# mnhrk15/integrated_path_planning

Hardware: AMD Instinct MI355X
Metric: candidate trajectories/sec (higher is better)
Workload: dtype f64; 1 GPU; config4: 256 ego instances/GPU x 2240-candidate lattice (5 s, dt 0.1 s), 20-sample x 30-pedestrian x 51-step fp32 prediction distribution (layout [S][P][T][2]), eps=0; 8 distinct batches rotated (501 MB of obstacle tensors per GPU); instances_per_gpu=256, instances_total=256, rotation_batches=8, plan_calls_in_flight=4

## Files before the change

### integrated_path_planning_amd/csrc/fot_kernels.hip

```cpp
#include <hip/hip_runtime.h>

#include <cstdlib>
#include <cstring>

#include "fot_math.hpp"
#include "fot_kernels.h"

namespace fot {


template <int CTRL, int ROW_MASK>
__device__ __forceinline__ float dpp_f32(float v)
{
    return __int_as_float(__builtin_amdgcn_update_dpp(__float_as_int(v), __float_as_int(v), CTRL, ROW_MASK, 0xf, false));
}

#define FOT_WAVE_REDUCE_F32(NAME, OP)                                                        \
    __device__ __forceinline__ float NAME(float v)                                           \
    {                                                                                        \
        v = OP(v, dpp_f32<0xB1, 0xf>(v));                           \
        v = OP(v, dpp_f32<0x4E, 0xf>(v));                           \
        v = OP(v, dpp_f32<0x141, 0xf>(v));                              \
        v = OP(v, dpp_f32<0x140, 0xf>(v));                                   \
        v = OP(v, dpp_f32<0x142, 0xa>(v));                     \
        v = OP(v, dpp_f32<0x143, 0xc>(v));                     \
        return __int_as_float(__builtin_amdgcn_readlane(__float_as_int(v), 63));             \
    }
FOT_WAVE_REDUCE_F32(wave_min_f32, fminf)
FOT_WAVE_REDUCE_F32(wave_max_f32, fmaxf)


__device__ __forceinline__ ScanBest wave_argmin(ScanBest b)
{
#pragma unroll
    for (int off = 32; off >= 1; off >>= 1) {
        ScanBest o;
        o.dist = __shfl_xor(b.dist, off, WAVE);
        o.idx = __shfl_xor(b.idx, off, WAVE);
        scan_merge(b, o);
    }
    return b;
}

template <typename T>
__device__ __forceinline__ T load_const(const T *table, int i)
{
    static_assert(sizeof(T) % sizeof(uint64_t) == 0, "copied in 8-byte words");
#if defined(__HIP_DEVICE_COMPILE__)
    typedef const __attribute__((address_space(4))) uint64_t const_u64;
    const_u64 *src = (const_u64 *)(table + i);
    T v;
#pragma unroll
    for (int k = 0; k < (int)(sizeof(T) / sizeof(uint64_t)); ++k) ((uint64_t *)&v)[k] = src[k];
    return v;
#else
    return table[i];
#endif
}

extern __shared__ double s_spl[];
constexpr int SPLINE_LDS_KNOTS = 512;

__device__ __forceinline__ void stage_spline_copy(const SplineView &g, double *s_spl)
{
    const double *src[9] = { g.s, g.ax, g.bx, g.cx, g.dx, g.ay, g.by, g.cy, g.dy };
    for (int i = threadIdx.x; i < 9 * g.n; i += blockDim.x) {
        const int a = i / g.n, j = i - a * g.n;
        s_spl[i] = src[a][j];
    }
}

__device__ __forceinline__ SplineView staged_spline_view(const SplineView &g, double *s_spl)
{
    SplineView l = g;
    l.s = s_spl; l.ax = s_spl + g.n; l.bx = s_spl + 2 * g.n; l.cx = s_spl + 3 * g.n; l.dx = s_spl + 4 * g.n;
    l.ay = s_spl + 5 * g.n; l.by = s_spl + 6 * g.n; l.cy = s_spl + 7 * g.n; l.dy = s_spl + 8 * g.n;
    return l;
}

__device__ __forceinline__ SplineView stage_spline(const SplineView &g, int lds_knots, double *s_spl = fot::s_spl)
{
    if (g.n > lds_knots) return g;
    stage_spline_copy(g, s_spl);
    __syncthreads();
    return staged_spline_view(g, s_spl);
}

__device__ __forceinline__ void refine_apply(int outcome, double s_end, double &s, double &ds)
{
    if (outcome == 0) s = fmax(0.0, s - ds);
    else if (outcome == 1) s = fmin(s_end, s + ds);
    else ds *= 0.5;
}

__device__ __forceinline__ double refine_nearest_wave(const SplineView &sp, double x, double y, double best_s, int lane)
{
    const double s_end = sp.s[sp.n - 1];
    int depth = 0, o1 = 0, o2 = 0, pos = lane;
    if (lane >= 12) { const int i = lane - 12; depth = 2; o1 = i / 9; o2 = (i / 3) % 3; pos = i % 3; }
    else if (lane >= 3) { const int i = lane - 3; depth = 1; o1 = i / 3; pos = i % 3; }
    if (lane >= 39) { depth = 0; pos = 1; }
    double ds = 0.2;
    for (int it = 0; it < 20; it += 3) {
        double ms = best_s, mds = ds;
        if (depth >= 1) refine_apply(o1, s_end, ms, mds);
        if (depth >= 2) refine_apply(o2, s_end, ms, mds);
        const double probe = pos == 0 ? fmax(0.0, ms - mds) : (pos == 1 ? ms : fmin(s_end, ms + mds));
        double px, py;
        spline_xy(sp, probe, px, py);
        const double dist = hypot_cr(x - px, y - py);
        const int rounds = 20 - it < 3 ? 20 - it : 3;
        int base = 0, r1 = 0;
// ... 1051 lines not shown
    if ((int)blockIdx.x < a.n_inst) {
        select_instance_wave((int)blockIdx.x, (int)threadIdx.x);
        record_written((int)blockIdx.x, (int)threadIdx.x);
    }
}

#define FOT_EVAL_LEAN false
#define FOT_EVAL_KERNEL(name) name
#include "fot_eval_kernels.inc"
#undef FOT_EVAL_LEAN
#undef FOT_EVAL_KERNEL
#define FOT_EVAL_LEAN true
#define FOT_EVAL_KERNEL(name) name##_lean
#include "fot_eval_kernels.inc"
#undef FOT_EVAL_LEAN
#undef FOT_EVAL_KERNEL


#ifndef FOT_CULL_KG
#define FOT_CULL_KG 4
#endif
constexpr int CULL_KG = FOT_CULL_KG;
constexpr int CULL_LIST = 256;
constexpr int CULL_PBOX = 96;
constexpr uint32_t CULL_IDX_MASK = 0xFFFFFu;
constexpr int CULL_VER = 256;
constexpr int CULL_BAD = 32;
constexpr uint32_t CULL_DEAD = 0xFFFFFFFFu;

template <typename T, int KG>
__device__ __forceinline__ void
cull_group(const DevParams *__restrict__ Pp, const InstDesc *__restrict__ desc, const InstState *__restrict__ state,
           const SplineView &sp, double *dyn_lds, const T *__restrict__ static_xy, const T *__restrict__ dyn_xy,
           int32_t *__restrict__ ent_cnt, f2 *__restrict__ ent32, d2 *__restrict__ ent64, uint8_t *__restrict__ ent_sid,
           TileStep *__restrict__ wave_rng, const int32_t *__restrict__ tile_cand0, const int32_t *__restrict__ tile_n,
           const int32_t *__restrict__ tile_span, const uint8_t *__restrict__ nan_flag, int ablate, int inst, int k0)
{
    __shared__ int s_cnt[KG][CULL_BINS + 1];
    __shared__ int s_start[KG][CULL_BINS + 1];
    __shared__ int s_nin[KG];
    __shared__ uint32_t s_list[KG][CULL_LIST];
    __shared__ uint32_t s_ver[CULL_VER];
    __shared__ uint32_t s_bad[CULL_BAD];
    __shared__ int s_nver, s_nbad;
    __shared__ Box32 s_box[KG];
    __shared__ BinMap s_bm[KG];
    __shared__ float s_margin[KG];
    __shared__ Box32 s_pbox[KG][CULL_PBOX];
    __shared__ LonQuartic s_linfo[CULL_PBOX];
    __shared__ uint8_t s_lext[CULL_PBOX];
    const DevParams &P = *Pp;
    const int n_ext_cap = P.n_ti + P.n_brake;
    double *s_ext = dyn_lds;
    double *s_latq = s_ext + KG * n_ext_cap * 2;
    const InstDesc &D = desc[inst];
    const InstState &S = state[inst];
    if (D.ent_cap == 0) return;
    const int tid = threadIdx.x, lane = tid & (WAVE - 1);
    const int wv = __builtin_amdgcn_readfirstlane(tid / WAVE);
    const int nk = P.n_total - k0 < KG ? P.n_total - k0 : KG;
    const int n_grid_lon = P.n_ti * D.n_tv;
    const int n_prof = S.c2f_ok ? n_grid_lon + S.n_brake : 0;
    const double sq_dyn = D.dyn_mode == FOT_DYN_SINGLE ? P.sq_r_dyn : P.sq_r;
    const double sq_max = sq_dyn > P.sq_r ? sq_dyn : P.sq_r;
    const FilterConst fc = filter_const(sq_max, sq_dyn < P.sq_r ? sq_dyn : P.sq_r);
    const float slack = box_footprint_slack(P);
    const int n_ext = P.n_ti + (S.c2f_ok ? S.n_brake : 0);
    for (int w = tid; w < n_prof && w < CULL_PBOX; w += KG * WAVE) {
        s_linfo[w] = lon_quartic(profile_info(P, D, S.frenet0, w, false));
        s_lext[w] = (uint8_t)extent_index(P, D, w);
    }
    if (S.c2f_ok && tid < n_ext) {
        const bool brake = tid >= P.n_ti;
        lateral_extent_coeffs(P, S.frenet0, brake, brake ? P.brake[tid - P.n_ti] : P.ti[tid], s_latq + tid * 9);
    }
    __syncthreads();
    if (ablate & 16) return;

    struct Raw { T x, y; };
    const bool dyn_on = D.dyn_mode != FOT_DYN_NONE;
    const int n_dyn = dyn_on ? D.S * D.P : 0;
    const int total = D.n_static + n_dyn;
    const bool tmajor = D.dyn_tmajor != 0;

    const int kl = tmajor ? wv : (lane & (KG - 1));
    const int i_first = tmajor ? lane : wv * (WAVE / KG) + lane / KG;
    constexpr int STRIDE = WAVE;
    const int row_l = k0 + kl < D.T - 1 ? k0 + kl : D.T - 1;
    auto fetch = [&](int i, Raw &o) {
        const int ic = i < total ? i : total - 1;
        const int j = ic - D.n_static;
        const T *ps = static_xy + 2 * ((int64_t)D.static_off + ic);
        const T *pd = dyn_xy + 2 * (D.dyn_off + (tmajor ? (int64_t)row_l * n_dyn + j : (int64_t)j * D.T + row_l));
        const Raw *src = (const Raw *)(ic < D.n_static ? ps : pd);
        o = *src;
    };
    if (!(ablate & 8)) {
        for (int i = tid; i < nk * n_ext; i += KG * WAVE) {
            const int ks = i / n_ext, e = i - ks * n_ext;
            const bool brake = e >= P.n_ti;
            const int n_eval = brake ? P.brake[e - P.n_ti].n_t : P.ti[e].n_t;
            double *ext = s_ext + (ks * n_ext_cap + e) * 2;
            lateral_extent_q(s_latq + e * 9, brake, k0 + ks, n_eval, P.dt, ext[0], ext[1]);
        }
        __syncthreads();
        const int n_tab = n_prof < CULL_PBOX ? n_prof : CULL_PBOX;
        for (int i = tid; i < nk * n_tab; i += KG * WAVE) {
            const int ks = i / n_tab, w = i - ks * n_tab;
            const double *ext = s_ext + (ks * n_ext_cap + s_lext[w]) * 2;
            s_pbox[ks][w] = profile_box_from(s_linfo[w], D, sp, k0 + ks, P.dt, ext[0], ext[1]);
        }
        __syncthreads();
    }
    {
        Box32 bw = box_empty();
        if (wv < nk && !(ablate & 8)) {
            for (int w = lane; w < n_prof; w += WAVE) {
                if (w < CULL_PBOX) {
                    box_merge(bw, s_pbox[wv][w]);
                } else {
                    const double *ext = s_ext + (wv * n_ext_cap + extent_index(P, D, w)) * 2;
                    box_merge(bw, profile_box_at(P, D, S.frenet0, sp, w, k0 + wv, ext[0], ext[1]));
                }
            }
        }
        bw.x0 = wave_min_f32(bw.x0); bw.y0 = wave_min_f32(bw.y0);
        bw.x1 = wave_max_f32(bw.x1); bw.y1 = wave_max_f32(bw.y1);
        const float mw = cull_margin(sq_max, bw) + slack;
        if (lane == 0) { s_box[wv] = bw; s_margin[wv] = mw; s_bm[wv] = bin_map(bw, mw); s_nin[wv] = 0; }
        if (lane <= CULL_BINS) s_cnt[wv][lane] = 0;
        if (tid == 0) { s_nver = 0; s_nbad = 0; }
    }
    __syncthreads();

    const bool lazy = dyn_on && !tmajor && !(ablate & 128);
    const Raw *tracks = (const Raw *)(dyn_xy + 2 * D.dyn_off);
    auto track_has_nan = [&](int j) {
        bool bad = false;
        for (int t = 0; t < D.T; ++t) { const Raw p = tracks[(int64_t)j * D.T + t]; bad |= (p.x != p.x) | (p.y != p.y); }
        return bad;
    };
    auto track_bad = [&](int i) {
        if (i < D.n_static) return false;
        return lazy ? track_has_nan(i - D.n_static) : nan_flag[D.nan_off + (i - D.n_static)] != 0;
    };

    {
        const Box32 bl = s_box[kl];
        const float ml = s_margin[kl];
        const BinMap bml = s_bm[kl];
        const bool live_l = kl < nk && bl.x0 <= bl.x1 && !(ablate & 4);
        auto classify = [&](int i, const Raw &o) {
            const float fx = (float)((double)o.x - D.ego.x), fy = (float)((double)o.y - D.ego.y);
            const bool in = i < total && live_l && cull_inside(bl, ml, fx, fy);
            if (lazy) {
                const uint64_t m = __ballot(in && i >= D.n_static);
                if ((lane & (KG - 1)) == 0 && ((m >> lane) & ((1ull << KG) - 1ull)) != 0ull) {
                    const int v = atomicAdd(&s_nver, 1);
                    if (v < CULL_VER) s_ver[v] = (uint32_t)i;
                }
                if (in) {
                    const int j = atomicAdd(&s_nin[kl], 1);
                    if (j < CULL_LIST) s_list[kl][j] = (uint32_t)i | ((uint32_t)bin_of(bml, fx, fy) << 20);
                }
                return;
            }
            if (in) {
                if (i >= D.n_static && nan_flag[D.nan_off + (i - D.n_static)]) return;
                const int bin = bin_of(bml, fx, fy);
                atomicAdd(&s_cnt[kl][bin], 1);
                const int j = atomicAdd(&s_nin[kl], 1);
                if (j < CULL_LIST) s_list[kl][j] = (uint32_t)i | ((uint32_t)bin << 20);
            }
        };
#ifndef FOT_CULL_UNROLL
#define FOT_CULL_UNROLL 4
#endif
        constexpr int UNROLL = FOT_CULL_UNROLL;
        if (ablate & 64) {
        } else if (D.n_static == 0) {
            const char *p0 = (const char *)(dyn_xy + 2 * (D.dyn_off + (tmajor ? (int64_t)row_l * n_dyn + i_first
                                                                              : (int64_t)i_first * D.T + row_l)));
            const int64_t step = (int64_t)(tmajor ? STRIDE : STRIDE * D.T) * (int64_t)(2 * sizeof(T));
            const char *p = p0;
            for (int ib = i_first; ib < total; ib += UNROLL * STRIDE) {
                Raw o[UNROLL];
#pragma unroll
                for (int u = 0; u < UNROLL; ++u) {
                    o[u] = *(const Raw *)(ib + u * STRIDE < total ? p : p0);
                    p += step;
                }
#pragma unroll
                for (int u = 0; u < UNROLL; ++u) classify(ib + u * STRIDE, o[u]);
            }
        } else {
            for (int ib = i_first; ib < total; ib += UNROLL * STRIDE) {
                Raw o[UNROLL];
#pragma unroll
                for (int u = 0; u < UNROLL; ++u) fetch(ib + u * STRIDE, o[u]);
#pragma unroll
                for (int u = 0; u < UNROLL; ++u) classify(ib + u * STRIDE, o[u]);
            }
        }
    }
    __syncthreads();
    if (lazy) {
#ifndef FOT_CULL_VU
#define FOT_CULL_VU 4
#endif
        constexpr int VU = FOT_CULL_VU;
        const int n_ver = s_nver < CULL_VER ? s_nver : CULL_VER;
        for (int v0 = wv; v0 < n_ver; v0 += VU * KG) {
            Raw p[VU];
#pragma unroll
            for (int u = 0; u < VU; ++u) {
                const int v = v0 + u * KG < n_ver ? v0 + u * KG : v0;
                p[u] = tracks[(int64_t)((int)s_ver[v] - D.n_static) * D.T + (lane < D.T ? lane : D.T - 1)];
            }
#pragma unroll
            for (int u = 0; u < VU; ++u) {
                const int v = v0 + u * KG;
                if (v >= n_ver) break;
                bool bad = (p[u].x != p[u].x) | (p[u].y != p[u].y);
                for (int t = WAVE + lane; t < D.T; t += WAVE) {
                    const Raw q = tracks[(int64_t)((int)s_ver[v] - D.n_static) * D.T + t];
                    bad |= (q.x != q.x) | (q.y != q.y);
                }
                if (__ballot(bad) != 0ull && lane == 0) {
                    const int nb = atomicAdd(&s_nbad, 1);
                    if (nb < CULL_BAD) s_bad[nb] = s_ver[v];
                }
            }
        }
        __syncthreads();
    }
    if (wv >= nk) return;
    const int kk = wv, k = k0 + wv;
    const bool listed = !lazy || (s_nin[kk] <= CULL_LIST && s_nver <= CULL_VER && s_nbad <= CULL_BAD);
    const Box32 bk = s_box[kk];
    const BinMap bmk = s_bm[kk];
    const float mk = s_margin[kk];
    const bool live_k = bk.x0 <= bk.x1;
    const int row = k < D.T - 1 ? k : D.T - 1;
    auto point = [&](int i, d2 &o, int &sid) {
        sid = SID_STATIC;
        if (i < D.n_static) {
            const int64_t in = D.static_off + i;
            o.x = (double)static_xy[2 * in]; o.y = (double)static_xy[2 * in + 1];
        } else {
            const int j = i - D.n_static;
            const int64_t in = D.dyn_off + (tmajor ? (int64_t)row * n_dyn + j : (int64_t)j * D.T + row);
            o.x = (double)dyn_xy[2 * in]; o.y = (double)dyn_xy[2 * in + 1];
            sid = j / D.P;
        }
    };
    if (lazy) {
        if (listed) {
            const int n_bad = s_nbad;
            for (int j = lane; j < s_nin[kk]; j += WAVE) {
                const uint32_t e = s_list[kk][j];
                bool bad = false;
                for (int b = 0; b < n_bad; ++b) bad |= s_bad[b] == (e & CULL_IDX_MASK);
                if (bad) s_list[kk][j] = CULL_DEAD;
                else atomicAdd(&s_cnt[kk][e >> 20], 1);
            }
        } else {
            for (int i0 = 0; i0 < total; i0 += WAVE) {
                const int i = i0 + lane;
                if (i >= total) continue;
                d2 o; int sid;
                point(i, o, sid);
                const float fx = (float)(o.x - D.ego.x), fy = (float)(o.y - D.ego.y);
                if (live_k && cull_inside(bk, mk, fx, fy) && !track_bad(i)) atomicAdd(&s_cnt[kk][bin_of(bmk, fx, fy)], 1);
            }
        }
        __builtin_amdgcn_fence(__ATOMIC_SEQ_CST, "wavefront");
        __builtin_amdgcn_wave_barrier();
    }
    {
        const int c = lane < CULL_BINS ? s_cnt[kk][lane] : 0;
        int incl = c;
#pragma unroll
        for (int off = 1; off < WAVE; off <<= 1) {
            const int t = __shfl_up(incl, off, WAVE);
            if (lane >= off) incl += t;
        }
        if (lane <= CULL_BINS) { s_start[kk][lane] = incl - c; s_cnt[kk][lane] = incl - c; }
    }
    __builtin_amdgcn_fence(__ATOMIC_SEQ_CST, "wavefront");
    __builtin_amdgcn_wave_barrier();
    const int64_t base = D.ent_off + (int64_t)k * D.ent_cap;
    TileStep *rng = wave_rng + (int64_t)D.tile0 * P.n_total + k;
    const int count = s_start[kk][CULL_BINS];
    if (lazy ? listed : count <= CULL_LIST) {
        for (int j = lane; j < ((ablate & 2) ? 0 : (lazy ? s_nin[kk] : count)); j += WAVE) {
            const uint32_t e = s_list[kk][j];
            if (e == CULL_DEAD) continue;
            const int i = (int)(e & CULL_IDX_MASK), bin = (int)(e >> 20);
            d2 o; int sid;
            point(i, o, sid);
            const int pos = atomicAdd(&s_cnt[kk][bin], 1);
            ent32_store(ent32, base + pos, (float)(o.x - D.ego.x), (float)(o.y - D.ego.y));
            ent64[base + pos] = o;
            ent_sid[base + pos] = (uint8_t)sid;
        }
    } else {
        for (int i0 = 0; i0 < total; i0 += WAVE) {
            const int i = i0 + lane;
            if (i >= total) continue;
            d2 o; int sid;
            point(i, o, sid);
            const float fx = (float)(o.x - D.ego.x), fy = (float)(o.y - D.ego.y);
            if (live_k && cull_inside(bk, mk, fx, fy) && !track_bad(i)) {
                const int bin = bin_of(bmk, fx, fy);
                const int pos = atomicAdd(&s_cnt[kk][bin], 1);
                ent32_store(ent32, base + pos, fx, fy);
                ent64[base + pos] = o;
                ent_sid[base + pos] = (uint8_t)sid;
            }
        }
    }
    const int padded = (count + 2 * ENT_CHUNK - 1) & ~(2 * ENT_CHUNK - 1);
    if (lane < padded - count) {
        d2 o; o.x = INFINITY; o.y = INFINITY;
        ent32_store(ent32, base + count + lane, FAR32, FAR32);
        ent64[base + count + lane] = o;
        ent_sid[base + count + lane] = SID_STATIC;
    }
    if (lane == 0) ent_cnt[(int64_t)inst * P.n_total + k] = padded;
    for (int w = lane; w < D.n_tiles; w += WAVE) {
        TileStep r = { 0u, 0.0f, 0.0f, 0u };
        const int idx0 = tile_cand0[D.shape_off + w];
        if (live_k && idx0 < S.n_cand && tile_n[D.shape_off + w] > 0 && !(ablate & 1)) {
            const uint32_t sp01 = (uint32_t)tile_span[D.shape_off + w];
            const int s0 = (int)(sp01 >> 16), s1 = (int)(sp01 & 0xffffu) < n_prof - 1 ? (int)(sp01 & 0xffffu) : n_prof - 1;
            Box32 wb = box_empty();
            for (int sl = s0; sl <= s1; ++sl) {
                if (sl < CULL_PBOX) { box_merge(wb, s_pbox[kk][sl]); continue; }
                const double *ext = s_ext + (kk * n_ext_cap + extent_index(P, D, sl)) * 2;
                box_merge(wb, profile_box_at(P, D, S.frenet0, sp, sl, k, ext[0], ext[1]));
            }
            const float wm = cull_margin(sq_max, wb) + slack;
            r.rng = strip_range(bmk, wb, wm, [&](int bb) { return s_start[kk][bb]; });
            box_thresholds(fc, wb, wm, r.thr, r.thr_sure);
        }
        rng[(int64_t)w * P.n_total] = r;
    }
}

template <typename T>
__global__ void __launch_bounds__(CULL_KG * WAVE)
k_cull(const DevParams *__restrict__ Pp, const InstDesc *__restrict__ desc, const InstState *__restrict__ state,
       int n_inst, SplineView sp_hbm, const SplineView *__restrict__ sp_table, int mixed, int lds_knots,
       const T *__restrict__ static_xy, const T *__restrict__ dyn_xy,
       int32_t *__restrict__ ent_cnt, f2 *__restrict__ ent32, d2 *__restrict__ ent64, uint8_t *__restrict__ ent_sid,
       TileStep *__restrict__ wave_rng, const int32_t *__restrict__ tile_cand0, const int32_t *__restrict__ tile_n,
       const int32_t *__restrict__ tile_span, const uint8_t *__restrict__ nan_flag,
       int ablate)
{
    if (ablate & 32) return;
    const int groups = (Pp->n_total + CULL_KG - 1) / CULL_KG;
    const int xcd = blockIdx.x & 7, seq = blockIdx.x >> 3;
    const int inst = xcd + 8 * (seq / groups), k0 = (seq % groups) * CULL_KG;
    if (inst >= n_inst) return;
    if (mixed) { Pp += desc[inst].scen; sp_hbm = load_const(sp_table, desc[inst].scen); }
    const SplineView sp = stage_spline(sp_hbm, lds_knots);
    cull_group<T, CULL_KG>(Pp, desc, state, sp, s_spl + 9 * lds_knots, static_xy, dyn_xy, ent_cnt, ent32, ent64, ent_sid,
                           wave_rng, tile_cand0, tile_n, tile_span, nan_flag, ablate, inst, k0);
}
// ... 309 lines not shown
```

### integrated_path_planning_amd/csrc/fot_math.hpp

```cpp
#pragma once

#include <math.h>
#include "fot_types.h"

namespace fot {


FOT_HD double fast_rcp(double a)
{
#if defined(__HIP_DEVICE_COMPILE__)
    double x = __builtin_amdgcn_rcp(a);
    x = fma(x, fma(-a, x, 1.0), x);
#ifdef FOT_NEWTON2
    x = fma(x, fma(-a, x, 1.0), x);
#endif
    return x;
#else
    return 1.0 / a;
#endif
}

FOT_HD double fast_rsqrt(double a)
{
#if defined(__HIP_DEVICE_COMPILE__)
// ... 879 lines not shown
    d1 = d0;
    if (!brake) {
        lat_coeffs(fr, (double)(P.n_di - 1 - P.n_side) * P.d_road_w, ti, q);
        lat_sample(q, k, n_eval, P.dt, d1, u0, u1, u2);
    }
}

FOT_HD void lateral_extent_q(const double *q9, bool brake, int k, int n_eval, double dt, double &d0, double &d1)
{
    double u0, u1, u2;
    lat_sample(q9, k, n_eval, dt, d0, u0, u1, u2);
    d1 = d0;
    if (!brake) {
        const double q_hi[6] = { q9[0], q9[1], q9[2], q9[6], q9[7], q9[8] };
        lat_sample(q_hi, k, n_eval, dt, d1, u0, u1, u2);
    }
}

FOT_HD void lateral_extent_coeffs(const DevParams &P, const double *fr, bool brake, const TimeInfo &ti, double *q9)
{
    double q_hi[6];
    lat_coeffs(fr, brake ? fr[3] : -(double)P.n_side * P.d_road_w, ti, q9);
    lat_coeffs(fr, brake ? fr[3] : (double)(P.n_di - 1 - P.n_side) * P.d_road_w, ti, q_hi);
    q9[6] = q_hi[3]; q9[7] = q_hi[4]; q9[8] = q_hi[5];
}

FOT_HD Box32 segment_box(double rx, double ry, double cos_r, double sin_r, double d0, double d1, double ox, double oy)
{
    Box32 b = box_empty();
    const double x0 = rx - sin_r * d0, y0 = ry + cos_r * d0, x1 = rx - sin_r * d1, y1 = ry + cos_r * d1;
    if (x0 == x0 && y0 == y0) box_add(b, (float)(x0 - ox), (float)(y0 - oy));
    if (x1 == x1 && y1 == y1) box_add(b, (float)(x1 - ox), (float)(y1 - oy));
    return b;
}

FOT_HD Box32 profile_box(const DevParams &P, const double *fr, bool brake, const TimeInfo &ti, const LonSample &ls,
                         int k, int n_eval, double ox, double oy)
{
    double d0, d1;
    lateral_extent(P, fr, brake, ti, k, n_eval, d0, d1);
    return segment_box(ls.rx, ls.ry, ls.cos_r, ls.sin_r, d0, d1, ox, oy);
}

FOT_HD Box32 profile_box_at(const DevParams &P, const InstDesc &D, const double *fr, const SplineView &sp, int slot,
                            int k, double d0, double d1)
{
    const LonInfo L = profile_info(P, D, fr, slot, false);
    if (k >= L.n_t) return box_empty();
    double s_, u0, u1, u2;
    lon_sample(L, k, P.dt, s_, u0, u1, u2);
    SplinePt p;
    spline_point(sp, s_, p);
    const double inv = fast_rsqrt(p.dx * p.dx + p.dy * p.dy);
    return segment_box(p.x, p.y, p.dx * inv, p.dy * inv, d0, d1, D.ego.x, D.ego.y);
}

struct LonQuartic {
    double a0, a1, a2, a3, a4;
    int32_t n_t, n_eval;
};

FOT_HD LonQuartic lon_quartic(const LonInfo &L)
{
    LonQuartic q;
    q.a0 = L.a0; q.a1 = L.a1; q.a2 = L.a2; q.a3 = L.a3; q.a4 = L.a4; q.n_t = L.n_t; q.n_eval = L.n_eval;
    return q;
}

FOT_HD Box32 profile_box_from(const LonQuartic &Q, const InstDesc &D, const SplineView &sp, int k, double dt, double d0,
                              double d1)
{
    if (k >= Q.n_t) return box_empty();
    LonInfo L;
    L.a0 = Q.a0; L.a1 = Q.a1; L.a2 = Q.a2; L.a3 = Q.a3; L.a4 = Q.a4; L.n_t = Q.n_t; L.n_eval = Q.n_eval;
    L.Js = 0.0; L.sd_last = 0.0; L.T = 0.0;
    double s_, u0, u1, u2;
    lon_sample(L, k, dt, s_, u0, u1, u2);
    SplinePt p;
    spline_point(sp, s_, p);
    const double inv = fast_rsqrt(p.dx * p.dx + p.dy * p.dy);
    return segment_box(p.x, p.y, p.dx * inv, p.dy * inv, d0, d1, D.ego.x, D.ego.y);
}

FOT_HD int extent_index(const DevParams &P, const InstDesc &D, int slot)
{
    const int n_grid_lon = P.n_ti * D.n_tv;
    return slot < n_grid_lon ? slot / D.n_tv : P.n_ti + (slot - n_grid_lon);
}

FOT_HD float box_footprint_slack(const DevParams &P)
{
    float m = 0.0f;
    if (P.has_footprint)
        for (int c = 0; c < P.n_circ; ++c) m = fmaxf(m, (float)fabs(P.circ_off[c]) * 1.000001f);
    return m;
}

constexpr int CULL_BINS = 32;
constexpr int ENT_CHUNK_ = 8;

struct BinMap {
    int axis;
    float lo, inv_w;
};

FOT_HD BinMap bin_map(const Box32 &b, float margin)
{
    BinMap m;
    m.axis = (b.y1 - b.y0) > (b.x1 - b.x0) ? 1 : 0;
    const float lo = (m.axis ? b.y0 : b.x0) - margin, hi = (m.axis ? b.y1 : b.x1) + margin;
    m.lo = lo;
    m.inv_w = (float)CULL_BINS / fmaxf(hi - lo, 1e-6f);
    return m;
}

FOT_HD int bin_of_value(const BinMap &m, float v)
{
    const float t = (v - m.lo) * m.inv_w;
    return t >= (float)(CULL_BINS - 1) ? CULL_BINS - 1 : (t > 0.0f ? (int)t : 0);
}

FOT_HD int bin_of(const BinMap &m, float x, float y) { return bin_of_value(m, m.axis ? y : x); }

template <class StartFn>
FOT_HD uint32_t strip_range(const BinMap &m, const Box32 &wb, float margin, const StartFn &bin_start)
{
    if (!(wb.x0 <= wb.x1)) return 0u;
    const float lo = (m.axis ? wb.y0 : wb.x0) - margin, hi = (m.axis ? wb.y1 : wb.x1) + margin;
    const int b_lo = bin_of_value(m, lo), b_hi = bin_of_value(m, hi);
    const int e_lo = bin_start(b_lo), e_hi = bin_start(b_hi + 1);
    if (e_hi <= e_lo) return 0u;
    const int c_lo = e_lo / ENT_CHUNK_, c_hi = (e_hi + ENT_CHUNK_ - 1) / ENT_CHUNK_;
    return ((uint32_t)c_lo << 16) | (uint32_t)c_hi;
}

FOT_HD void wave_profile_span(const DevParams &P, const InstDesc &D, int n_tv_grid_lon, int idx0, int idx1,
                              int &first, int &last)
{
    const int per_prof = P.n_di;
    first = idx0 < D.n_grid ? idx0 / per_prof : n_tv_grid_lon + (idx0 - D.n_grid);
    last = idx1 < D.n_grid ? idx1 / per_prof : n_tv_grid_lon + (idx1 - D.n_grid);
}

constexpr int ENT_CHUNK = 8;
static_assert(ENT_CHUNK == 8, "strip_range assumes 8-entry chunks");
constexpr int SID_STATIC = 255;
struct alignas(64) f2x8 { float x[ENT_CHUNK]; float y[ENT_CHUNK]; };

FOT_HD void ent32_store(f2 *e32, int64_t pos, float x, float y)
{
    f2x8 *c = (f2x8 *)e32 + (pos >> 3);
    c->x[pos & 7] = x;
    c->y[pos & 7] = y;
}

FOT_HD float min_sqdist32_8(const f2x8 &c, float fx, float fy)
{
    float t[ENT_CHUNK];
    for (int j = 0; j < ENT_CHUNK; ++j) {
        const float dx = fx - c.x[j], dy = fy - c.y[j];
        t[j] = fmaf(dy, dy, dx * dx);
    }
    float m = fminf(fminf(t[0], t[1]), t[2]);
    m = fminf(fminf(m, t[3]), t[4]);
    m = fminf(fminf(m, t[5]), t[6]);
    return fminf(m, t[7]);
}

struct FilterConst { float sq, r, sq_lo; };

FOT_HD FilterConst filter_const(double sq, double sq_min)
// ... 472 lines not shown
```

### integrated_path_planning_amd/csrc/fot_setup.hpp

```cpp
#pragma once

#include <algorithm>
#include <cmath>
#include <cstring>
#include <string>
#include <cstdlib>
#include <vector>

#include "fot_types.h"
#include "fot_math.hpp"

namespace fot {


inline bool time_info(double T, double dt, TimeInfo &ti)
{
    ti.T = T;
    ti.n_t = (int)std::nearbyint(T / dt) + 1;
    if (ti.n_t < 1 || ti.n_t > FOT_MAX_NT) return false;
    const double T2 = T * T, T3 = T2 * T, T4 = T2 * T2, T5 = T4 * T;
    {
        const double a = 3.0 * T2, b = 4.0 * T3, c = 6.0 * T, d = 12.0 * T2;
        const double det = a * d - b * c;
        ti.qa[0] = d / det; ti.qa[1] = -b / det; ti.qa[2] = -c / det; ti.qa[3] = a / det;
// ... 331 lines not shown
    L.n_inst = b.n_inst;
    L.desc.resize(b.n_inst);
    L.grouped = sc[0].shapes->grouped;
    for (int s = 0; s < n_scen; ++s)
        if (sc[s].shapes->row_budget > L.row_budget) L.row_budget = sc[s].shapes->row_budget;
    std::vector<uint8_t> used((size_t)n_scen, 0);
    for (int i = 0; i < b.n_inst; ++i) {
        InstDesc &D = L.desc[i];
        D = InstDesc();
        D.ego = b.ego[i];
        const int si = scen ? scen[i] : 0;
        if (si < 0 || si >= n_scen) { err = "unknown scenario id"; return FOT_ERR_INVALID; }
        const fot_params &hp = *sc[si].hp;
        const DevParams &P = *sc[si].P;
        const TileShapes &shapes = *sc[si].shapes;
        D.scen = si;
        used[(size_t)si] = 1;
        if (D.ego.has_prev_s < 0 || D.ego.has_prev_s > FOT_EGO_IS_FRENET) { err = "has_prev_s must be 0 .. 3"; return FOT_ERR_INVALID; }
        if (i == 0 && D.ego.has_prev_s == FOT_PREV_S_CHAINED) { err = "the first instance cannot be chained"; return FOT_ERR_INVALID; }
        if (i > 0 && D.ego.has_prev_s == FOT_PREV_S_CHAINED && si != L.desc[i - 1].scen) {
            err = "a chained instance must be on its predecessor's scenario (a chain is one planner)"; return FOT_ERR_INVALID;
        }
        const double target = b.target_speed[i];
        D.target_speed = target;
        D.max_stop = b.max_stop_distance ? b.max_stop_distance[i] : NAN;
        D.lim_speed = hp.max_speed; D.lim_accel = hp.max_accel; D.lim_curv = hp.max_curvature; D.lim_lat = hp.max_lat_accel;
        if (b.overrides) {
            const fot_overrides &o = b.overrides[i];
            if (!std::isnan(o.max_speed)) D.lim_speed = o.max_speed;
            if (!std::isnan(o.max_accel)) D.lim_accel = o.max_accel;
            if (!std::isnan(o.max_curvature)) D.lim_curv = o.max_curvature;
            if (!std::isnan(o.max_lat_accel)) D.lim_lat = o.max_lat_accel;
        }
        D.step_limit = std::fmax(D.lim_speed, hp.max_speed) * hp.dt * 3.0;

        if (!std::isfinite(target)) { err = "target_speed must be finite"; return FOT_ERR_INVALID; }
        const int n_down = (int)(target / hp.d_t_s + 1e-9);
        if (n_down + 1 <= 0) { err = "target_speed too negative: empty terminal-speed grid"; return FOT_ERR_INVALID; }
        const double tv_last = target - (double)n_down * hp.d_t_s;
        D.n_down = n_down;
        D.n_tv = n_down + 1 + (tv_last > 1e-9 ? 1 : 0);
        if (D.n_tv > FOT_MAX_TV) { err = "terminal-speed grid larger than FOT_MAX_TV"; return FOT_ERR_UNSUPPORTED; }
        D.n_grid = P.n_ti * D.n_tv * P.n_di;
        D.n_cand_max = D.n_grid + P.n_brake;

        const int n_tiles_i = shapes.tiles_of(D.n_tv);
        D.shape_off = sc[si].shape_base + shapes.off[D.n_tv];
        const int64_t slots_i = ((int64_t)D.n_cand_max + WAVE - 1) / WAVE * WAVE;
        if (L.n_slots + slots_i > 0x7fffffffLL || (int64_t)L.n_tiles + n_tiles_i > 0x7fffffffLL) {
            err = "batch too large"; return FOT_ERR_UNSUPPORTED;
        }
        D.cand_off = (int32_t)L.n_slots;
        D.tile0 = L.n_tiles;
        D.n_tiles = n_tiles_i;
        L.n_tiles += n_tiles_i;
        if (n_tiles_i > L.max_tiles) L.max_tiles = n_tiles_i;
        L.n_slots += slots_i;
        const int n_lon_i = P.n_ti * D.n_tv + P.n_brake;
        D.lon_off = (int32_t)L.n_lon;
        L.n_lon += n_lon_i;
        if (n_lon_i > L.max_lon) L.max_lon = n_lon_i;

        if (b.static_off) {
            const int64_t lo = b.static_off[i], hi = b.static_off[i + 1];
            if (lo < 0 || hi < lo) { err = "static_off must be non-decreasing"; return FOT_ERR_INVALID; }
            D.static_off = lo;
            D.n_static = (int32_t)(hi - lo);
            if (hi > L.n_static) L.n_static = hi;
        }
        D.dyn_mode = FOT_DYN_NONE;
        if (b.dyn_off && b.dyn_dims) {
            const int32_t *dm = b.dyn_dims + 4 * i;
            const int mode = dm[0] & ~FOT_DYN_LAYOUT_TSP;
            D.dyn_tmajor = (dm[0] & FOT_DYN_LAYOUT_TSP) ? 1 : 0;
            int S = dm[1], Pn = dm[2], T = dm[3];
            if (mode != FOT_DYN_NONE && mode != FOT_DYN_SINGLE && mode != FOT_DYN_DISTRIBUTION) {
                err = "dyn_dims mode"; return FOT_ERR_INVALID;
            }
            if (mode == FOT_DYN_SINGLE) S = 1;
            if (mode != FOT_DYN_NONE && S > 0 && Pn > 0 && T > 0) {
                if (S > FOT_MAX_SAMPLES) { err = "more prediction samples than FOT_MAX_SAMPLES"; return FOT_ERR_UNSUPPORTED; }
                if (b.dyn_off[i] < 0) { err = "dyn_off < 0"; return FOT_ERR_INVALID; }
                D.dyn_mode = mode; D.S = S; D.P = Pn; D.T = T;
                if (D.dyn_tmajor) L.any_tmajor = true;
                D.dyn_off = b.dyn_off[i];
                const int64_t pts = (int64_t)S * Pn * T;
                if (D.dyn_off + pts > L.dyn_src_points) L.dyn_src_points = D.dyn_off + pts;
                D.max_viol = mode == FOT_DYN_DISTRIBUTION ? (int)std::floor(hp.chance_epsilon * (double)S) : 0;
                D.nan_off = L.n_tracks;
                L.n_tracks += ((int64_t)S * Pn + 15) & ~(int64_t)15;
                const int64_t bytes = pts * 2 * (b.obstacle_dtype == FOT_F32 ? 4 : 8);
                if (bytes > L.max_dyn_bytes) L.max_dyn_bytes = bytes;
            }
        }
        const int64_t per_k = (int64_t)D.n_static + (D.dyn_mode != FOT_DYN_NONE ? (int64_t)D.S * D.P : 0);
        if (per_k > 0) {
            if (per_k > 65534 * 8) { err = "too many obstacle points in one instance"; return FOT_ERR_UNSUPPORTED; }
            D.ent_cap = (int32_t)((per_k + 15) & ~(int64_t)15);
            D.ent_off = L.n_entries;
            L.n_entries += (int64_t)D.ent_cap * P.n_total;
            L.any_obstacles = true;
        }
    }
    for (int i = b.n_inst - 1, run = 0; i >= 0; --i) {
        L.desc[i].n_chained = run;
        run = L.desc[i].ego.has_prev_s == FOT_PREV_S_CHAINED ? run + 1 : 0;
    }
    if ((L.n_static > 0 && !b.static_xy) || (L.dyn_src_points > 0 && !b.dyn_xy)) {
        err = "obstacle offsets given without coordinates";
        return FOT_ERR_INVALID;
    }
    for (int s = 0; s < n_scen; ++s)
        if (used[(size_t)s]) {
            L.scens.push_back(s);
            const int e = sc[s].P->n_ti + sc[s].P->n_brake;
            if (e > L.n_ext) L.n_ext = e;
        }
    return FOT_OK;
}

inline int build_batch_layout(const fot_params &hp, const DevParams &P, const TileShapes &shapes, const fot_batch &b,
                              BatchLayout &L, std::string &err)
{
    ScenarioRef one;
    one.hp = &hp; one.P = &P; one.shapes = &shapes; one.shape_base = 0;
    return build_batch_layout(&one, 1, nullptr, b, L, err);
}

}
```

### integrated_path_planning_amd/csrc/fot_types.h

```cpp
#pragma once

#include <stddef.h>
#include <stdint.h>
#include "../../include/fot.h"

#if defined(__HIPCC__) || defined(__HIP__)
#define FOT_HD __host__ __device__ __forceinline__
#else
#define FOT_HD inline
#endif

namespace fot {

constexpr int WAVE = 64;
constexpr int WAVES_PER_GROUP = 4;
constexpr int TILE_MAX_PROFILES = 8;
constexpr int N_XCD = 8;
constexpr int LON_FIELDS = 10;
constexpr int ST_PENDING = FOT_ST_OK;

struct d2 { double x, y; };
struct f2 { float x, y; };
constexpr float FAR32 = 1.0e18f;

struct TimeInfo {
    double T;
    double qa[4];
    double qi[9];
    int32_t n_t;
    int32_t _pad;
};

struct DevParams {
    double max_speed, max_accel, max_curvature, max_lat_accel;
    double dt, d_road_w, max_road_width, min_t, d_t_s;
    double k_j, k_t, k_d, k_s_dot, k_lat, k_lon;
    double sq_r, sq_r_dyn;
    double chance_epsilon;
    double road_lim;
    double circ_off[FOT_MAX_CIRCLES];
    int32_t n_ti, n_di, n_side, n_brake;
    int32_t n_total;
    int32_t n_circ;
    int32_t has_footprint;
    int32_t _pad;
    TimeInfo ti[FOT_MAX_TI];
    TimeInfo brake[FOT_MAX_BRAKE];
};

struct SplineView {
    const double *s, *ax, *bx, *cx, *dx, *ay, *by, *cy, *dy;
    int32_t n;
    int32_t _pad;
};

struct InstDesc {
    fot_ego ego;
    double target_speed;
    double max_stop;
    double lim_speed, lim_accel, lim_curv, lim_lat;
    double step_limit;
    int32_t n_tv;
    int32_t n_down;
    int32_t n_grid;
    int32_t cand_off;
    int32_t n_cand_max;
    int32_t lon_off;
    int32_t n_static;
    int64_t static_off;
    int32_t dyn_mode, S, P, T;
    int64_t dyn_off;
    int64_t ent_off;
    int32_t ent_cap;
    int32_t tile0;
    int32_t n_tiles;
    int32_t shape_off;
    int32_t dyn_tmajor;
    int32_t max_viol;
    int32_t n_chained;
    int32_t scen;
    int64_t nan_off;
};

struct InstState {
    double frenet0[6];
    double ref0[6];
    double new_prev_s;
    int32_t c2f_ok;
    int32_t n_brake;
    int32_t n_cand;
    int32_t _pad;
};

struct LonInfo {
    double a0, a1, a2, a3, a4;
    double Js;
    double sd_last;
    double T;
    int32_t n_t;
    int32_t n_eval;
};

constexpr int GROUP_HEAD_TILES = 4, GROUP_HEAD_PROFILES = 16;
enum : int32_t {
    GROUP_HEAD_ABSENT = 0,
    GROUP_HEAD_EMPTY = 2,
    GROUP_HEAD_FULL = 1
};
struct alignas(128) GroupHead {
    int32_t present;
    int32_t grp_tile0;
    int32_t slot_lo, n_stage;
    int32_t total_rows;
    int32_t n_total, n_circ_fp;
    int32_t cand_off, tile0, ent_cap, max_viol;
    int32_t n_grid, n_tv, n_di, n_side, n_ti;
    int32_t row0[GROUP_HEAD_PROFILES + 1];
    int32_t t_cand0[GROUP_HEAD_TILES], t_n[GROUP_HEAD_TILES];
    int32_t t_n_loop[GROUP_HEAD_TILES];
    int32_t t_own_lo[GROUP_HEAD_TILES], t_own_hi[GROUP_HEAD_TILES];
    int64_t ent_off;
    double d_road_w, dt, road_lim;
    double lim_speed, lim_accel, lim_curv, lim_lat;
    double ego_x, ego_y;
    double frenet0[6];
    LonInfo info[GROUP_HEAD_PROFILES];
};
static_assert(sizeof(GroupHead) % 128 == 0 && sizeof(GroupHead) == 1536, "whole 128-byte lines");

constexpr int HEAD_COMMON_DWORDS = 344 / 4;
enum : int32_t { HEAD_VARIANT_GRID = 0, HEAD_VARIANT_BRAKE = 1, HEAD_VARIANTS = 2 };
struct HeadProfile {
    int32_t ti, itv;
    int32_t n_t, n_eval;
    double T;
};
struct alignas(128) HeadTemplate {
    uint32_t common[HEAD_COMMON_DWORDS];
    uint32_t _pad[2];
    HeadProfile prof[GROUP_HEAD_PROFILES];
};
static_assert(sizeof(HeadTemplate) == 768, "whole 128-byte lines");
static_assert(offsetof(GroupHead, info) == 4 * HEAD_COMMON_DWORDS, "HeadTemplate::common is the GroupHead in front of info");

}
```

Measured before the change: 2.834 billion candidates/s.

## Micro-optimize cull kernel: 32-bit offsets, DPP reductions, magic division, spline index guess

Bundles several micro-optimizations in the obstacle culling kernel: 32-bit byte offsets for dynamic obstacle loads when the tensor fits, inline-asm DPP min/max reductions without NaN handling, a DPP prefix sum replacing shuffle-based scan, magic-number division for the sample id, compare-based small quotients, a guessed uniform-spacing spline index before falling back to search, and a ballot-based leader election. The aim is fewer integer, address and VALU instructions in the hot cull path. The changes add complexity and depend on assumptions such as offsets fitting in 31 bits and inputs being NaN-free in the reductions.

```diff
diff --git a/integrated_path_planning_amd/csrc/fot_kernels.hip b/integrated_path_planning_amd/csrc/fot_kernels.hip
--- a/integrated_path_planning_amd/csrc/fot_kernels.hip
+++ b/integrated_path_planning_amd/csrc/fot_kernels.hip
@@ -28,6 +28,33 @@
     }
 FOT_WAVE_REDUCE_F32(wave_min_f32, fminf)
 FOT_WAVE_REDUCE_F32(wave_max_f32, fmaxf)
+
+#define FOT_WAVE_REDUCE_F32_ASM(NAME, OP)                                                    \
+    __device__ __forceinline__ float NAME(float v)                                           \
+    {                                                                                        \
+        asm("s_nop 1\n\t"                                                                    \
+            OP " %0, %0, %0 quad_perm:[1,0,3,2] row_mask:0xf bank_mask:0xf\n\ts_nop 1\n\t"   \
+            OP " %0, %0, %0 quad_perm:[2,3,0,1] row_mask:0xf bank_mask:0xf\n\ts_nop 1\n\t"   \
+            OP " %0, %0, %0 row_half_mirror row_mask:0xf bank_mask:0xf\n\ts_nop 1\n\t"       \
+            OP " %0, %0, %0 row_mirror row_mask:0xf bank_mask:0xf\n\ts_nop 1\n\t"            \
+            OP " %0, %0, %0 row_bcast:15 row_mask:0xa bank_mask:0xf\n\ts_nop 1\n\t"          \
+            OP " %0, %0, %0 row_bcast:31 row_mask:0xc bank_mask:0xf\n\ts_nop 1"              \
+            : "+v"(v));                                                                      \
+        return __int_as_float(__builtin_amdgcn_readlane(__float_as_int(v), 63));             \
+    }
+FOT_WAVE_REDUCE_F32_ASM(wave_min_nonan_f32, "v_min_f32_dpp")
+FOT_WAVE_REDUCE_F32_ASM(wave_max_nonan_f32, "v_max_f32_dpp")
+
+__device__ __forceinline__ int wave_prefix_sum_i32(int v)
+{
+    v += __builtin_amdgcn_update_dpp(0, v, 0x111, 0xf, 0xf, false);
+    v += __builtin_amdgcn_update_dpp(0, v, 0x112, 0xf, 0xf, false);
+    v += __builtin_amdgcn_update_dpp(0, v, 0x114, 0xf, 0xf, false);
+    v += __builtin_amdgcn_update_dpp(0, v, 0x118, 0xf, 0xf, false);
+    v += __builtin_amdgcn_update_dpp(0, v, 0x142, 0xa, 0xf, false);
+    v += __builtin_amdgcn_update_dpp(0, v, 0x143, 0xc, 0xf, false);
+    return v;
+}
 
 
 __device__ __forceinline__ ScanBest wave_argmin(ScanBest b)
@@ -1245,6 +1272,11 @@
     const int n_dyn = dyn_on ? D.S * D.P : 0;
     const int total = D.n_static + n_dyn;
     const bool tmajor = D.dyn_tmajor != 0;
+    const char *dyn_base = (const char *)(dyn_xy + 2 * D.dyn_off);
+    const bool off32 = offsets_fit32((int64_t)n_dyn * D.T * (int64_t)sizeof(Raw));
+    auto dyn_offset = [&](int j, int row) {
+        return (uint32_t)(tmajor ? row * n_dyn + j : j * D.T + row) * (uint32_t)sizeof(Raw);
+    };
 
     const int kl = tmajor ? wv : (lane & (KG - 1));
     const int i_first = tmajor ? lane : wv * (WAVE / KG) + lane / KG;
@@ -1254,13 +1286,14 @@
         const int ic = i < total ? i : total - 1;
         const int j = ic - D.n_static;
         const T *ps = static_xy + 2 * ((int64_t)D.static_off + ic);
-        const T *pd = dyn_xy + 2 * (D.dyn_off + (tmajor ? (int64_t)row_l * n_dyn + j : (int64_t)j * D.T + row_l));
+        const T *pd = off32 ? (const T *)(dyn_base + dyn_offset(j, row_l))
+                            : dyn_xy + 2 * (D.dyn_off + (tmajor ? (int64_t)row_l * n_dyn + j : (int64_t)j * D.T + row_l));
         const Raw *src = (const Raw *)(ic < D.n_static ? ps : pd);
         o = *src;
     };
     if (!(ablate & 8)) {
         for (int i = tid; i < nk * n_ext; i += KG * WAVE) {
-            const int ks = i / n_ext, e = i - ks * n_ext;
+            const int ks = small_quotient(i, n_ext, KG), e = i - ks * n_ext;
             const bool brake = e >= P.n_ti;
             const int n_eval = brake ? P.brake[e - P.n_ti].n_t : P.ti[e].n_t;
             double *ext = s_ext + (ks * n_ext_cap + e) * 2;
@@ -1268,10 +1301,11 @@
         }
         __syncthreads();
         const int n_tab = n_prof < CULL_PBOX ? n_prof : CULL_PBOX;
+        const float sp_scale = spline_guess_scale(sp);
         for (int i = tid; i < nk * n_tab; i += KG * WAVE) {
-            const int ks = i / n_tab, w = i - ks * n_tab;
+            const int ks = small_quotient(i, n_tab, KG), w = i - ks * n_tab;
             const double *ext = s_ext + (ks * n_ext_cap + s_lext[w]) * 2;
-            s_pbox[ks][w] = profile_box_from(s_linfo[w], D, sp, k0 + ks, P.dt, ext[0], ext[1]);
+            s_pbox[ks][w] = profile_box_from_guess(s_linfo[w], D, sp, sp_scale, k0 + ks, P.dt, ext[0], ext[1]);
         }
         __syncthreads();
     }
@@ -1287,8 +1321,8 @@
                 }
             }
         }
-        bw.x0 = wave_min_f32(bw.x0); bw.y0 = wave_min_f32(bw.y0);
-        bw.x1 = wave_max_f32(bw.x1); bw.y1 = wave_max_f32(bw.y1);
+        bw.x0 = wave_min_nonan_f32(bw.x0); bw.y0 = wave_min_nonan_f32(bw.y0);
+        bw.x1 = wave_max_nonan_f32(bw.x1); bw.y1 = wave_max_nonan_f32(bw.y1);
         const float mw = cull_margin(sq_max, bw) + slack;
         if (lane == 0) { s_box[wv] = bw; s_margin[wv] = mw; s_bm[wv] = bin_map(bw, mw); s_nin[wv] = 0; }
         if (lane <= CULL_BINS) s_cnt[wv][lane] = 0;
@@ -1300,6 +1334,7 @@
     const Raw *tracks = (const Raw *)(dyn_xy + 2 * D.dyn_off);
     auto track_has_nan = [&](int j) {
         bool bad = false;
+#pragma clang loop vectorize(disable) unroll(disable)
         for (int t = 0; t < D.T; ++t) { const Raw p = tracks[(int64_t)j * D.T + t]; bad |= (p.x != p.x) | (p.y != p.y); }
         return bad;
     };
@@ -1317,8 +1352,11 @@
             const float fx = (float)((double)o.x - D.ego.x), fy = (float)((double)o.y - D.ego.y);
             const bool in = i < total && live_l && cull_inside(bl, ml, fx, fy);
             if (lazy) {
-                const uint64_t m = __ballot(in && i >= D.n_static);
-                if ((lane & (KG - 1)) == 0 && ((m >> lane) & ((1ull << KG) - 1ull)) != 0ull) {
+                uint64_t m = __builtin_amdgcn_ballot_w64(in && i >= D.n_static);
+#pragma unroll
+                for (int s = 1; s < KG; s <<= 1) m |= m >> s;
+                constexpr uint64_t FIRST = ~0ull / ((1ull << KG) - 1ull);
+                if (__builtin_amdgcn_inverse_ballot_w64(m & FIRST)) {
                     const int v = atomicAdd(&s_nver, 1);
                     if (v < CULL_VER) s_ver[v] = (uint32_t)i;
                 }
@@ -1341,6 +1379,21 @@
 #endif
         constexpr int UNROLL = FOT_CULL_UNROLL;
         if (ablate & 64) {
+        } else if (D.n_static == 0 && off32) {
+            const uint32_t step = (uint32_t)(tmajor ? STRIDE : STRIDE * D.T) * (uint32_t)sizeof(Raw);
+            const uint32_t o_last = (uint32_t)((int64_t)n_dyn * D.T * (int64_t)sizeof(Raw)) - (uint32_t)sizeof(Raw);
+            uint32_t off = dyn_offset(i_first, row_l);
+            for (int ib = i_first; ib < total; ib += UNROLL * STRIDE) {
+                Raw o[UNROLL];
+#pragma unroll
+                for (int u = 0; u < UNROLL; ++u) {
+                    const uint32_t ou = off + (uint32_t)u * step;
+                    o[u] = *(const Raw *)(dyn_base + (ou < o_last ? ou : o_last));
+                }
+                off += (uint32_t)UNROLL * step;
+#pragma unroll
+                for (int u = 0; u < UNROLL; ++u) classify(ib + u * STRIDE, o[u]);
+            }
         } else if (D.n_static == 0) {
             const char *p0 = (const char *)(dyn_xy + 2 * (D.dyn_off + (tmajor ? (int64_t)row_l * n_dyn + i_first
                                                                               : (int64_t)i_first * D.T + row_l)));
@@ -1378,7 +1431,9 @@
 #pragma unroll
             for (int u = 0; u < VU; ++u) {
                 const int v = v0 + u * KG < n_ver ? v0 + u * KG : v0;
-                p[u] = tracks[(int64_t)((int)s_ver[v] - D.n_static) * D.T + (lane < D.T ? lane : D.T - 1)];
+                const int j = (int)s_ver[v] - D.n_static, t = lane < D.T ? lane : D.T - 1;
+                p[u] = off32 ? *(const Raw *)(dyn_base + (uint32_t)(j * D.T + t) * (uint32_t)sizeof(Raw))
+                             : tracks[(int64_t)j * D.T + t];
             }
 #pragma unroll
             for (int u = 0; u < VU; ++u) {
@@ -1412,9 +1467,14 @@
             o.x = (double)static_xy[2 * in]; o.y = (double)static_xy[2 * in + 1];
         } else {
             const int j = i - D.n_static;
-            const int64_t in = D.dyn_off + (tmajor ? (int64_t)row * n_dyn + j : (int64_t)j * D.T + row);
-            o.x = (double)dyn_xy[2 * in]; o.y = (double)dyn_xy[2 * in + 1];
-            sid = j / D.P;
+            if (off32) {
+                const Raw r = *(const Raw *)(dyn_base + dyn_offset(j, row));
+                o.x = (double)r.x; o.y = (double)r.y;
+            } else {
+                const int64_t in = D.dyn_off + (tmajor ? (int64_t)row * n_dyn + j : (int64_t)j * D.T + row);
+                o.x = (double)dyn_xy[2 * in]; o.y = (double)dyn_xy[2 * in + 1];
+            }
+            sid = (int)div_by_magic((uint32_t)j, (uint32_t)D.P, D.p_magic);
         }
     };
     if (lazy) {
@@ -1423,6 +1483,7 @@
             for (int j = lane; j < s_nin[kk]; j += WAVE) {
                 const uint32_t e = s_list[kk][j];
                 bool bad = false;
+#pragma clang loop vectorize(disable) unroll(disable)
                 for (int b = 0; b < n_bad; ++b) bad |= s_bad[b] == (e & CULL_IDX_MASK);
                 if (bad) s_list[kk][j] = CULL_DEAD;
                 else atomicAdd(&s_cnt[kk][e >> 20], 1);
@@ -1442,12 +1503,7 @@
     }
     {
         const int c = lane < CULL_BINS ? s_cnt[kk][lane] : 0;
-        int incl = c;
-#pragma unroll
-        for (int off = 1; off < WAVE; off <<= 1) {
-            const int t = __shfl_up(incl, off, WAVE);
-            if (lane >= off) incl += t;
-        }
+        const int incl = wave_prefix_sum_i32(c);
         if (lane <= CULL_BINS) { s_start[kk][lane] = incl - c; s_cnt[kk][lane] = incl - c; }
     }
     __builtin_amdgcn_fence(__ATOMIC_SEQ_CST, "wavefront");
diff --git a/integrated_path_planning_amd/csrc/fot_math.hpp b/integrated_path_planning_amd/csrc/fot_math.hpp
--- a/integrated_path_planning_amd/csrc/fot_math.hpp
+++ b/integrated_path_planning_amd/csrc/fot_math.hpp
@@ -985,11 +985,73 @@
     return segment_box(p.x, p.y, p.dx * inv, p.dy * inv, d0, d1, D.ego.x, D.ego.y);
 }
 
+FOT_HD float spline_guess_scale(const SplineView &sp)
+{
+    const float len = (float)(sp.s[sp.n - 1] - sp.s[0]);
+#if defined(__HIP_DEVICE_COMPILE__)
+    return (float)(sp.n - 1) * __builtin_amdgcn_rcpf(len);
+#else
+    return (float)(sp.n - 1) / len;
+#endif
+}
+
+FOT_HD int spline_index_guess(const SplineView &sp, double v, float inv_h)
+{
+    const float top = (float)(sp.n - 2);
+    float gf = (float)(v - sp.s[0]) * inv_h;
+    gf = gf >= 0.0f ? (gf <= top ? gf : top) : 0.0f;
+    const int g = (int)gf;
+    if (sp.s[g] <= v && v < sp.s[g + 1]) return g;
+    return spline_index(sp, v);
+}
+
+FOT_HD Box32 profile_box_from_guess(const LonQuartic &Q, const InstDesc &D, const SplineView &sp, float inv_h, int k,
+                                    double dt, double d0, double d1)
+{
+    if (k >= Q.n_t) return box_empty();
+    LonInfo L;
+    L.a0 = Q.a0; L.a1 = Q.a1; L.a2 = Q.a2; L.a3 = Q.a3; L.a4 = Q.a4; L.n_t = Q.n_t; L.n_eval = Q.n_eval;
+    L.Js = 0.0; L.sd_last = 0.0; L.T = 0.0;
+    double s_, u0, u1, u2;
+    lon_sample(L, k, dt, s_, u0, u1, u2);
+    double px = NAN, py = NAN, pdx = NAN, pdy = NAN;
+    if (s_ >= sp.s[0] && s_ <= sp.s[sp.n - 1]) {
+        const int i = spline_index_guess(sp, s_, inv_h);
+        const double h = s_ - sp.s[i], h2 = h * h;
+        const double bx = sp.bx[i], cx = sp.cx[i], dx = sp.dx[i];
+        const double by = sp.by[i], cy = sp.cy[i], dy = sp.dy[i];
+        px = sp.ax[i] + bx * h + cx * h2 + dx * (h2 * h);
+        py = sp.ay[i] + by * h + cy * h2 + dy * (h2 * h);
+        pdx = bx + 2.0 * cx * h + 3.0 * dx * h2;
+        pdy = by + 2.0 * cy * h + 3.0 * dy * h2;
+    }
+    const double inv = fast_rsqrt(pdx * pdx + pdy * pdy);
+    return segment_box(px, py, pdx * inv, pdy * inv, d0, d1, D.ego.x, D.ego.y);
+}
+
 FOT_HD int extent_index(const DevParams &P, const InstDesc &D, int slot)
 {
     const int n_grid_lon = P.n_ti * D.n_tv;
     return slot < n_grid_lon ? slot / D.n_tv : P.n_ti + (slot - n_grid_lon);
 }
+
+
+FOT_HD uint32_t div_magic(uint32_t d) { return d <= 1u ? 0xffffffffu : (uint32_t)(0x100000000ull / d); }
+
+FOT_HD uint32_t div_by_magic(uint32_t n, uint32_t d, uint32_t m)
+{
+    const uint32_t q = (uint32_t)(((uint64_t)n * m) >> 32);
+    return q + (n - q * d >= d ? 1u : 0u);
+}
+
+FOT_HD int small_quotient(int i, int n, int kg)
+{
+    int q = 0;
+    for (int m = 1; m < kg; ++m) q += i >= m * n ? 1 : 0;
+    return q;
+}
+
+FOT_HD bool offsets_fit32(int64_t bytes) { return bytes < ((int64_t)1 << 31); }
 
 FOT_HD float box_footprint_slack(const DevParams &P)
 {
diff --git a/integrated_path_planning_amd/csrc/fot_setup.hpp b/integrated_path_planning_amd/csrc/fot_setup.hpp
--- a/integrated_path_planning_amd/csrc/fot_setup.hpp
+++ b/integrated_path_planning_amd/csrc/fot_setup.hpp
@@ -437,6 +437,7 @@
                 if (S > FOT_MAX_SAMPLES) { err = "more prediction samples than FOT_MAX_SAMPLES"; return FOT_ERR_UNSUPPORTED; }
                 if (b.dyn_off[i] < 0) { err = "dyn_off < 0"; return FOT_ERR_INVALID; }
                 D.dyn_mode = mode; D.S = S; D.P = Pn; D.T = T;
+                D.p_magic = div_magic((uint32_t)Pn);
                 if (D.dyn_tmajor) L.any_tmajor = true;
                 D.dyn_off = b.dyn_off[i];
                 const int64_t pts = (int64_t)S * Pn * T;
diff --git a/integrated_path_planning_amd/csrc/fot_types.h b/integrated_path_planning_amd/csrc/fot_types.h
--- a/integrated_path_planning_amd/csrc/fot_types.h
+++ b/integrated_path_planning_amd/csrc/fot_types.h
@@ -67,6 +67,7 @@
     int32_t n_cand_max;
     int32_t lon_off;
     int32_t n_static;
+    uint32_t p_magic;
     int64_t static_off;
     int32_t dyn_mode, S, P, T;
     int64_t dyn_off;
```

Result: faster. 2.874 billion candidates/s (median of 6 runs) (+1.4%).
